# sony/NDJIR

Hardware: AMD Instinct MI355X
Metric: rays/sec (fwd+bwd) at 512 rays x 128 samples (higher is better)
Workload: dtype f32 (f16x2-split MFMA products, f32 accumulate; error vs fp64 below an fp32 FMA chain's)

## Files before the change

### include/ndjir_hip.h

```cpp
#ifndef NDJIR_HIP_H
#define NDJIR_HIP_H

#include <hip/hip_runtime_api.h>

#ifdef __cplusplus
extern "C" {
#endif

#define NDJIR_OK 0
#define NDJIR_ERR_LAUNCH 1
#define NDJIR_ERR_UNSUPPORTED 2
#define NDJIR_ERR_ARG 3

const char* ndjir_version(void);
int ndjir_zero(float* p, long long n, hipStream_t stream);

int ndjir_hash_force_align(int size, int mod);
int ndjir_hash_grid_size(int G0, float growth_factor, int level);
int ndjir_hash_table_size(int G, int T0);
long long ndjir_hash_num_params(int G0, float growth_factor, int T0, int L, int D);

#define NDJIR_DECL_VOXEL_FAMILY(P)                                                                                          \
  int ndjir_##P##_query_on_voxel(int N, float* output, const float* query, const float* feature, const int* grid_sizes,     \
                                 int D, const float* min, const float* max, int boundary_check, hipStream_t stream);       \
// ... 257 lines not shown

int ndjir_geo_encode(long long P, int M, const float* x, int nseg, const float* const* seg, const int* segC, float* e, int lde,
                     hipStream_t stream);
int ndjir_geo_normal(long long P, int M, const float* e, int lde, const float* g0, int ldg, int nseg, const float* const* gq,
                     float* n_out, float* Z, int ldz, int D, float* sdf_out, hipStream_t stream);
int ndjir_geo_backward_begin(long long P, int D, const float* g_sdf, const float* g_feat, int ldf, const float* g_n,
                             const float* gZ, int ldz, float* gy, float* nbar, hipStream_t stream);
int ndjir_geo_gbar0(long long P, int M, const float* e, int lde, const float* nbar, int nseg, const float* const* seg,
                    const int* segC, float* gb0, hipStream_t stream);
int ndjir_copy_columns(long long P, int C, const float* src, int lds, float* dst, int ldd, hipStream_t stream);
int ndjir_inverse_squared_distance(long long P, long long rows_per_batch, const float* x, int ldx, const float* camloc, float* out,
                                   int ldo, hipStream_t stream);

int ndjir_mlp_chain_group_begin(void);
int ndjir_mlp_chain_group_end(hipStream_t stream, int* launches);

#define NDJIR_MATH_FP32 0
#define NDJIR_MATH_BF16X6 1
#define NDJIR_MATH_F16X3 2
int ndjir_mlp_set_math(int math);
int ndjir_mlp_get_math(void);
int ndjir_mlp_set_tile_rows(int rows);
int ndjir_mlp_get_tile_rows(void);
int ndjir_mlp_small_affine(long long P, const float* x, int ldx, int K, const float* W, int ldw, int N, int transpose,
                           const float* bias, float* y, int ldy, hipStream_t stream);
int ndjir_mlp_set_chain_pipeline(int mask);
int ndjir_mlp_get_chain_pipeline(void);
long long ndjir_mlp_packed_size(int K, int N, int transpose);
int ndjir_mlp_pack(const float* W, float* dst, int K, int N, int transpose, hipStream_t stream);
int ndjir_mlp_pack_strided(const float* W, int ldw, float* dst, int K, int N, int transpose, hipStream_t stream);
int ndjir_mlp_pack_table(const void* table, int n, int total_blocks, hipStream_t stream);
int ndjir_mlp_pack_entry_bytes(void);
int ndjir_mlp_chain(int bwd, long long P, const float* X, int ldx, int K0, int L,
                    const float* const* Wp, const float* const* bias, const int* Ks, const int* Ns,
                    const float* const* side_in, float* const* side_out, const int* ld_side,
                    float* const* bgrad, float* Y, int ldy, int accum_y, int has_output, float beta,
                    int skip_layer, float skip_scale, int skip_split, float* Xskip, int ld_xskip,
                    float* in_bgrad, float* workspace, unsigned* const* side_amax, unsigned* x_amax, hipStream_t stream);
long long ndjir_mlp_chain_workspace(int bgrad_total);
int ndjir_mlp_chain_ex(int mode, long long P, const float* X, int ldx, int K0, int L,
                       const float* const* Wp, const float* const* bias, const int* Ks, const int* Ns,
                       const float* const* side_in, float* const* side_out, const int* ld_side,
                       float* const* bgrad, float* Y, int ldy, int accum_y, int has_output, float beta,
                       int skip_layer, float skip_scale, int skip_split, float* Xskip, int ld_xskip,
                       const float* const* side_in2, const float* const* side_add, float* const* side_out2,
                       const float* row_bias, int row_bias_div, float* in_bgrad, float* workspace,
                       unsigned* const* side_amax, unsigned* x_amax, hipStream_t stream);
int ndjir_mlp_group_colsum(const float* X, int ldx, int N, long long G, int div, float* out, int blocked, hipStream_t stream);
long long ndjir_mlp_wgrad_workspace(int K, int N, long long P);
int ndjir_mlp_wgrad(const float* A, int lda, const float* B, int ldb, int K, int N, long long P, float* out,
                    int accum, float* workspace, const unsigned* amax_a, const unsigned* amax_b, hipStream_t stream);
long long ndjir_mlp_wgrad_group_workspace(int n_src, const float* const* A, const int* lda, const long long* P, const int* out_id,
                                          int n_out, const int* K, const int* N, int target_items, const int* layout);
int ndjir_mlp_wgrad_group_launches(int n_src, const long long* P, const int* out_id, int n_out);
int ndjir_mlp_wgrad_group(int n_src, const float* const* A, const int* lda, const float* const* B, const int* ldb,
                          const long long* P, const unsigned* const* amax_a, const unsigned* const* amax_b, const int* out_id,
                          int n_out, float* const* out, const int* ldo, const int* K, const int* N, const int* accum,
                          float* workspace, int target_items, int n_extra, float* const* ex_out, const float* const* ex_partial,
                          const int* ex_n, const int* ex_S, const int* ex_stride, const int* ex_accum, const int* layout,
                          hipStream_t stream);
long long ndjir_mlp_colsum_workspace(int N, long long P);
int ndjir_mlp_colsum(const float* X, int ldx, int N, long long P, float* out, int accum, float* workspace,
                     hipStream_t stream);
int ndjir_mlp_chain_kernel(int mode, long long P, int K0, int L, const int* Ks, const int* Ns, int has_output, int skip_layer,
                           int skip_split, int with_bias_gradients, char* name, int name_bytes);
int ndjir_mlp_chain_bias_partials(int mode, long long P, int K0, int L, const int* Ks, const int* Ns, int has_output,
                                  int skip_layer, int skip_split, unsigned bgrad_mask, int in_bgrad, int* blocks, int* row_floats);
int ndjir_mlp_debug_timeline(long long* buf);


int ndjir_generate_raydir_camloc(int B, int R, const double* pose, const double* intrinsic, const int* pixel_index,
                                 const float* xy, int W, float* raydir, float* camloc, hipStream_t stream);

typedef struct ndjir_adam_state { float alpha; int t; float alpha_t; int skipped; } ndjir_adam_state;
int ndjir_solver_adam_begin(void* state, float beta1, float beta2, const int* flag_a, const int* flag_b,
                            hipStream_t stream);
int ndjir_solver_adam(long long n, float* w, float* g, float* m, float* v, float alpha_t, float beta1, float beta2,
                      float eps, float decay, int zero_grad, const void* state, hipStream_t stream);
int ndjir_solver_adam_touched(long long n, float* w, float* g, float* m, float* v, float alpha_t, float beta1, float beta2,
                              float eps, float decay, unsigned* touched, const void* state, hipStream_t stream);
int ndjir_voxel_feature_mark_touched(int N, const float* query, const int* grid_sizes, int D, const float* min,
                                     const float* max, unsigned* bitmap, hipStream_t stream);
int ndjir_solver_adam_multi(int count, float* const* w, const float* const* g, float* const* m, float* const* v,
                            const long long* numel, float alpha_t, float beta1, float beta2, float eps, float decay,
                            const void* state, hipStream_t stream);
int ndjir_solver_check_inf_or_nan(long long n, const float* g, int* flag, hipStream_t stream);
int ndjir_solver_check_inf_or_nan_multi(int count, const float* const* g, const long long* numel, int* flag,
                                        hipStream_t stream);
// ... 8 lines not shown
```

### ndjir_amd/csrc/capi_mlp.hip

```cpp
#include <hip/hip_runtime.h>
#include <stdlib.h>

#include "../../include/ndjir_hip.h"
#include "common.h"
#include "mlp.h"

using namespace ndjir;

static inline int round_up(int v, int m) { return (v + m - 1) / m * m; }

static int g_math = NDJIR_MATH_F16X3;

extern "C" int ndjir_mlp_set_math(int math) {
  if (math != NDJIR_MATH_FP32 && math != NDJIR_MATH_BF16X6 && math != NDJIR_MATH_F16X3) return NDJIR_ERR_ARG;
  g_math = math;
  return NDJIR_OK;
}

extern "C" int ndjir_mlp_get_math(void) { return g_math; }

extern "C" long long ndjir_mlp_packed_size(int K, int N, int transpose) {
  if (g_math == NDJIR_MATH_BF16X6) return packed_size6(K, N, transpose);
  if (g_math == NDJIR_MATH_F16X3) return packed_size3(K, N, transpose);
  int Kp = round_up(transpose ? N : K, 8), Np = round_up(transpose ? K : N, 32);
// ... 28 lines not shown
static thread_local GroupCall* g_group = nullptr;
static thread_local int g_group_n = 0;
static thread_local int g_group_err = NDJIR_OK;
static thread_local ChainDry* g_dry = nullptr;

static int g_tile_rows = -1;
static int tile_rows_setting() {
  if (g_tile_rows < 0) { const char* e = getenv("NDJIR_MLP_TILE"); g_tile_rows = e ? atoi(e) : 0; }
  return g_tile_rows;
}
extern "C" int ndjir_mlp_set_tile_rows(int rows) {
  if (rows != 0 && rows != 32 && rows != 64 && rows != 128) return NDJIR_ERR_ARG;
  g_tile_rows = rows;
  return NDJIR_OK;
}
extern "C" int ndjir_mlp_get_tile_rows(void) { return tile_rows_setting(); }

extern "C" int ndjir_mlp_set_chain_pipeline(int mask) {
  if (mask < 0 || mask > 7) return NDJIR_ERR_ARG;
  chain_pipeline(mask);
  return NDJIR_OK;
}
extern "C" int ndjir_mlp_get_chain_pipeline(void) { return chain_pipeline(-1); }

static int chain_impl(int bwd, long long P, const float* X, int ldx, int K0, int L,
                               const float* const* Wp, const float* const* bias, const int* Ks, const int* Ns,
                               const float* const* side_in, float* const* side_out, const int* ld_side,
                               float* const* bgrad, float* Y, int ldy, int accum_y, int has_output, float beta,
                               int skip_layer, float skip_scale, int skip_split, float* Xskip, int ld_xskip,
                               const float* const* side_in2, const float* const* side_add, float* const* side_out2,
                               const float* row_bias, int row_bias_div, float* in_bgrad, float* workspace,
                               unsigned* const* side_amax, unsigned* x_amax, hipStream_t stream) {
  if (P <= 0) {
    if (bwd != 0 && in_bgrad && K0 > 0 && hipMemsetAsync(in_bgrad, 0, (size_t)K0 * sizeof(float), stream) != hipSuccess)
      return NDJIR_ERR_LAUNCH;
    if (bwd != 0 && bgrad && Ns && L >= 1 && L <= MAX_CHAIN_LAYERS)
      for (int i = 0; i < L; ++i)
        if (bgrad[i] && hipMemsetAsync(bgrad[i], 0, (size_t)Ns[i] * sizeof(float), stream) != hipSuccess) return NDJIR_ERR_LAUNCH;
    return NDJIR_OK;
  }
  if (!X || L < 1 || L > MAX_CHAIN_LAYERS || !Wp || !Ks || !Ns) return NDJIR_ERR_ARG;
  if (has_output && !Y) return NDJIR_ERR_ARG;
  ChainArgs a{};
  const int forced = tile_rows_setting();
  a.tile_rows = forced ? forced : ((P + 63) / 64 < 256 ? 32 : 64);
  a.forced_tile = forced;
// ... 101 lines not shown
                               float* in_bgrad, float* workspace, unsigned* const* side_amax, unsigned* x_amax,
                               hipStream_t stream) {
  if (bwd != 0 && bwd != 1) return NDJIR_ERR_ARG;
  return chain_impl(bwd, P, X, ldx, K0, L, Wp, bias, Ks, Ns, side_in, side_out, ld_side, bgrad, Y, ldy, accum_y,
                    has_output, beta, skip_layer, skip_scale, skip_split, Xskip, ld_xskip, nullptr, nullptr, nullptr, nullptr, 0,
                    in_bgrad, workspace, side_amax, x_amax, stream);
}

extern "C" int ndjir_mlp_chain_ex(int mode, long long P, const float* X, int ldx, int K0, int L,
                                  const float* const* Wp, const float* const* bias, const int* Ks, const int* Ns,
                                  const float* const* side_in, float* const* side_out, const int* ld_side,
                                  float* const* bgrad, float* Y, int ldy, int accum_y, int has_output, float beta,
                                  int skip_layer, float skip_scale, int skip_split, float* Xskip, int ld_xskip,
                                  const float* const* side_in2, const float* const* side_add, float* const* side_out2,
                                  const float* row_bias, int row_bias_div, float* in_bgrad, float* workspace,
                                  unsigned* const* side_amax, unsigned* x_amax, hipStream_t stream) {
  if (mode < 0 || mode > 2) return NDJIR_ERR_ARG;
  return chain_impl(mode, P, X, ldx, K0, L, Wp, bias, Ks, Ns, side_in, side_out, ld_side, bgrad, Y, ldy, accum_y,
                    has_output, beta, skip_layer, skip_scale, skip_split, Xskip, ld_xskip, side_in2, side_add, side_out2,
                    row_bias, row_bias_div, in_bgrad, workspace, side_amax, x_amax, stream);
}

static int chain_dry(int mode, long long P, int K0, int L, const int* Ks, const int* Ns, int has_output, int skip_layer,
                     int skip_split, unsigned bgrad_mask, int in_bgrad, ChainDry* out) {
  if (mode < 0 || mode > 2 || L < 1 || L > MAX_CHAIN_LAYERS || !Ks || !Ns || P <= 0) return NDJIR_ERR_ARG;
  static float dummy[4];
  const float* wp[MAX_CHAIN_LAYERS];
  const float* side[MAX_CHAIN_LAYERS];
  float* bg[MAX_CHAIN_LAYERS];
  for (int i = 0; i < L; ++i) { wp[i] = dummy; side[i] = dummy; bg[i] = (mode != 0 && ((bgrad_mask >> i) & 1)) ? dummy : nullptr; }
  out->name[0] = 0; out->blocks = 0; out->bg_total = 0;
  g_dry = out;
  const int rc = chain_impl(mode, P, dummy, K0, K0, L, wp, nullptr, Ks, Ns, mode != 0 ? side : nullptr, nullptr, nullptr,
                            mode != 0 ? bg : nullptr, dummy, Ns[L - 1], 0, has_output, 100.f, skip_layer, 1.f,
                            skip_split, (mode == 1 && skip_layer >= 0) ? dummy : nullptr, K0, nullptr, nullptr, nullptr, nullptr, 0,
                            (mode != 0 && in_bgrad) ? dummy : nullptr, dummy, nullptr, nullptr, nullptr);
  g_dry = nullptr;
  return rc;
}

extern "C" int ndjir_mlp_chain_kernel(int mode, long long P, int K0, int L, const int* Ks, const int* Ns, int has_output,
                                      int skip_layer, int skip_split, int with_bias_gradients, char* name, int name_bytes) {
  if (!name || name_bytes < 64) return NDJIR_ERR_ARG;
  ChainDry d;
  const int rc = chain_dry(mode, P, K0, L, Ks, Ns, has_output, skip_layer, skip_split, with_bias_gradients ? ~0u : 0u, 0, &d);
  for (int i = 0; i < 64; ++i) name[i] = d.name[i];
  return rc;
}

extern "C" int ndjir_mlp_chain_bias_partials(int mode, long long P, int K0, int L, const int* Ks, const int* Ns, int has_output,
                                             int skip_layer, int skip_split, unsigned bgrad_mask, int in_bgrad, int* blocks,
                                             int* row_floats) {
  if (!blocks || !row_floats) return NDJIR_ERR_ARG;
  ChainDry d;
  const int rc = chain_dry(mode, P, K0, L, Ks, Ns, has_output, skip_layer, skip_split, bgrad_mask, in_bgrad, &d);
  if (rc != NDJIR_OK) return rc;
  if (d.bg_total < 0) return NDJIR_ERR_UNSUPPORTED;
  *blocks = d.blocks;
  *row_floats = d.bg_total;
  return NDJIR_OK;
}

extern "C" long long ndjir_mlp_chain_workspace(int bgrad_total) { return chain_workspace(bgrad_total); }

extern "C" long long ndjir_mlp_wgrad_workspace(int K, int N, long long P) { return wgrad_workspace(K, N, P); }

extern "C" int ndjir_mlp_wgrad(const float* A, int lda, const float* B, int ldb, int K, int N, long long P, float* out,
                               int accum, float* workspace, const unsigned* amax_a, const unsigned* amax_b,
// ... 63 lines not shown
```

### ndjir_amd/csrc/mlp.h

```cpp
#pragma once
#include <hip/hip_runtime.h>

namespace ndjir {

constexpr int MAX_CHAIN_LAYERS = 10;

struct ChainLayer {
  const float* Wp;
  const float* bias;
  const float* side_in;
  const float* side_in2;
  const float* side_add;
  float* side_out2;
  float* side_out;
  float* bgrad;
  unsigned* side_amax;
  int bg_off;
  int K, N;
  int Kp, Np;
  int ld_side;
};

struct ChainDry {
  char name[64];
// ... 43 lines not shown
static_assert(sizeof(ChainGroup) <= 4096, "kernel arguments are limited to 4 KB");

int launch_pack(const float* W, float* dst, int K, int N, int transpose, hipStream_t stream);
int launch_chain(const ChainArgs& a, int mode, hipStream_t stream);
int launch_bgrad_reduce(const float* partial, int S, int total, float* const* ptr, const int* off, int n, int accum, hipStream_t stream);
long long packed_size6(int K, int N, int transpose);
int launch_pack6(const float* W, float* dst, int K, int N, int transpose, hipStream_t stream);
int launch_chain6(const ChainArgs& a, int mode, hipStream_t stream);
long long packed_size3(int K, int N, int transpose);
int launch_pack3(const float* W, int ldw, float* dst, int K, int N, int transpose, hipStream_t stream);
struct PackEntry {
  const float* W;
  float* dst;
  int K, N, ldw, transpose;
  int Kp, Np;
  int first_block;
  int pad;
};
int launch_pack3_table(const PackEntry* table, int n, int total_blocks, hipStream_t stream);
int launch_chain3(const ChainArgs& a, int mode, hipStream_t stream);
int launch_chainw(const ChainArgs& a, int mode, hipStream_t stream);
int launch_chainw_group(const ChainArgs* nets, int n, int mode, hipStream_t stream);
int chain_pipeline(int set);
constexpr int CHAIN_MAX_GRID_BG = 512;
inline long long chain_workspace(int bg_total) { return (long long)CHAIN_MAX_GRID_BG * ((bg_total + 3) & ~3); }
long long wgrad_workspace(int K, int N, long long P);
int launch_wgrad(const float* A, int lda, const float* B, int ldb, int K, int N, long long P, float* out, int accum,
                 float* workspace, int math, const unsigned* amax_a, const unsigned* amax_b, hipStream_t stream);

long long wgrad_group_workspace(int n_src, const float* const* A, const int* lda, const long long* P, const int* out_id, int n_out,
                                const int* K, const int* N, int target_items, const int* layout);
int wgrad_group_launches(int n_src, const long long* P, const int* out_id, int n_out);
int launch_wgrad_group(int n_src, const float* const* A, const int* lda, const float* const* B, const int* ldb, const long long* P,
                       const unsigned* const* amax_a, const unsigned* const* amax_b, const int* out_id, int n_out,
                       float* const* out, const int* ldo, const int* K, const int* N, const int* accum, float* workspace,
                       int target_items, int n_extra, float* const* ex_out, const float* const* ex_partial, const int* ex_n,
                       const int* ex_S, const int* ex_stride, const int* ex_accum, const int* layout, hipStream_t stream);

long long colsum_workspace(int N, long long P);
int launch_group_colsum(const float* X, int ldx, int N, long long G, int div, float* out, int blocked, hipStream_t stream);
int launch_colsum(const float* X, int ldx, int N, long long P, float* out, int accum, float* workspace,
                  hipStream_t stream);

}
```

### ndjir_amd/csrc/mlp3.hip

```cpp
#include <hip/hip_runtime.h>
#include <stdio.h>
#include <stdint.h>

#include <type_traits>

#include "common.h"
#include "mlp.h"
#include "mlp3_util.h"

namespace ndjir {
namespace x3 {

using namespace x3u;

constexpr int NWAVES = 8;
constexpr int NTHREADS = NWAVES * 64;
constexpr int MAXNB = 16;
constexpr int GPS = 32 * 4 + 4;
constexpr int STG = 8 * GPS;
constexpr int IN_CACHE = 10;
#ifndef NDJIR_BWD_KLOOP_BARRIER
#define NDJIR_BWD_KLOOP_BARRIER 0
#endif
constexpr bool BWD_KLOOP_BARRIER = NDJIR_BWD_KLOOP_BARRIER;
// ... 840 lines not shown

int launch_pack3_table(const PackEntry* table, int n, int total_blocks, hipStream_t stream) {
  if (n <= 0 || total_blocks <= 0) return NDJIR_OK;
  hipLaunchKernelGGL(x3::k_pack3_table, dim3(total_blocks), dim3(x3::PACK_T), 0, stream, table, n);
  return ndjir_check_launch();
}

int launch_chain3(const ChainArgs& a, int mode, hipStream_t stream) {
  using namespace x3;
  constexpr int LDS_DYN_MAX = 160 * 1024 - 2048;
  if (a.P <= 0) return NDJIR_OK;
  if (a.tile_rows == 128 || (a.tile_rows == 64 && a.forced_tile == 0)) {
    const int rc = launch_chainw(a, mode, stream);
    if (rc != NDJIR_ERR_UNSUPPORTED) return rc;
  }
  int TM = a.tile_rows == 32 ? 32 : 64;
  int wmax = round_up(a.K0, 16);
  for (int i = 0; i < a.L; ++i) {
    const bool last = a.has_output && i == a.L - 1;
    if (a.layers[i].Np > MAXNB * 32) return NDJIR_ERR_UNSUPPORTED;
    if (!last && a.layers[i].Np > NWAVES * 32) TM = 32;
    if (!last && a.layers[i].Np > 32) { if (a.layers[i].Np > wmax) wmax = a.layers[i].Np; }
  }
  const int TMP = TM + 4;
  if (a.skip_layer >= 0 && mode != 1) { int w = round_up(a.layers[a.skip_layer].N + a.K0, 16); if (w > wmax) wmax = w; }
  ChainArgs b = a;
  b.K0p = round_up(a.K0, 16);
  b.lds_split = (wmax / 8) * TMP;
  size_t lds_bytes = (size_t)2 * b.lds_split * 16;
  size_t stage_bytes = (size_t)NWAVES * 2 * STG * 4;
  const size_t partials = (size_t)4 * TM * 32 * 4;
  if (stage_bytes < partials) stage_bytes = partials;
  lds_bytes += stage_bytes;
  b.n_tiles = (a.P + TM - 1) / TM;
  float* bg_ptr[MAX_CHAIN_LAYERS + 1];
  int bg_off[MAX_CHAIN_LAYERS + 1];
  int bg_n = 0, bg_total = 0;
  if (mode != 0) {
    for (int i = 0; i < a.L; ++i) if (a.layers[i].bgrad && !(a.has_output && i == a.L - 1)) {
      b.layers[i].bg_off = bg_total;
      bg_ptr[bg_n] = a.layers[i].bgrad;
      bg_off[bg_n] = bg_total;
      ++bg_n;
      bg_total += a.layers[i].N;
    } else b.layers[i].bgrad = nullptr;
  }
// ... 36 lines not shown
```

### ndjir_amd/lib.py

```python
import ctypes
import os

import torch

_HERE = os.path.dirname(os.path.abspath(__file__))
SO_PATH = os.environ.get("NDJIR_HIP_LIB") or os.path.join(_HERE, "_lib", "libndjir_hip.so")

_vp = ctypes.c_void_p
_CT = {"i": ctypes.c_int, "f": ctypes.c_float, "p": _vp, "q": _vp, "F": ctypes.POINTER(ctypes.c_float),
       "I": ctypes.POINTER(ctypes.c_int), "l": ctypes.c_longlong, "P": ctypes.POINTER(_vp),
       "A": ctypes.POINTER(ctypes.c_int), "L": ctypes.POINTER(ctypes.c_longlong), "x": _vp,
       "W": ctypes.POINTER(ctypes.c_float)}

_VOX_TAIL, _PLN_TAIL, _HSH_TAIL = "IiFFi", "iiFFi", "ifiiiFFi"


def _family(prefix, fwd, tail):
    return {
        f"{prefix}_{fwd}": "ippp" + tail,
        f"{prefix}_grad_query": "ipppp" + tail + "i",
        f"{prefix}_grad_feature": "ippp" + tail + "i",
        f"{prefix}_grad_query_grad_grad_output": "ipppp" + tail + "i",
        f"{prefix}_grad_query_grad_feature": "ipppp" + tail + "i",
    }
# ... 206 lines not shown
            cargs.append(v.data_ptr())
        elif c == "W":
            cargs.append((ctypes.c_float * len(v))(*[float(x) for x in v]))
        elif c == "F":
            cargs.append(_f3(v))
        elif c == "I":
            cargs.append(_i3(v))
        elif c == "f":
            cargs.append(float(v))
        else:
            cargs.append(int(v))
    stream = torch.cuda.current_stream().cuda_stream
    rc = f(*cargs, stream)
    if rc != 0:
        raise NdjirHipError(f"ndjir_{name} failed with status {rc}")


def symbols():
    return ["ndjir_" + n for n in SIGS] + ["ndjir_version", "ndjir_hash_force_align", "ndjir_hash_grid_size",
                                            "ndjir_hash_table_size", "ndjir_hash_num_params",
                                            "ndjir_mlp_packed_size", "ndjir_mlp_wgrad_workspace", "ndjir_mlp_wgrad_group_workspace", "ndjir_mlp_wgrad_group_launches", "ndjir_mlp_colsum_workspace",
                                            "ndjir_mlp_chain_workspace", "ndjir_mlp_set_math", "ndjir_mlp_get_math",
                                            "ndjir_mlp_set_tile_rows", "ndjir_mlp_get_tile_rows", "ndjir_mlp_set_chain_pipeline", "ndjir_mlp_get_chain_pipeline", "ndjir_mlp_pack_entry_bytes",
                                            "ndjir_mlp_debug_timeline", "ndjir_mlp_chain_kernel", "ndjir_mlp_chain_bias_partials", "ndjir_loss_terms_workspace",
                                            "ndjir_mlp_chain_group_begin", "ndjir_mlp_chain_group_end", "ndjir_sparse_rows_header"]


def hash_num_params(G0, growth_factor, T0, L, D):
    return int(load().ndjir_hash_num_params(int(G0), float(growth_factor), int(T0), int(L), int(D)))
```

### ndjir_amd/mlp.py

```python
import contextlib
import os
import weakref


import torch
from torch.autograd import Function
from torch.multiprocessing.reductions import StorageWeakRef as _StorageRef

from . import lib
from .registry import REG

_PACK_CACHE = REG.pack_cache

MATH_FP32, MATH_BF16X6, MATH_F16X3 = 0, 1, 2


def set_math(math):
    if lib.load().ndjir_mlp_set_math(int(math)) != 0:
        raise lib.NdjirHipError(f"unknown math mode {math}")
    _PACK_CACHE.clear()


def get_math():
    return int(lib.load().ndjir_mlp_get_math())


def set_tile_rows(rows):
    if lib.load().ndjir_mlp_set_tile_rows(int(rows)) != 0:
        raise ValueError(f"tile rows {rows}")


def get_tile_rows():
    return int(lib.load().ndjir_mlp_get_tile_rows())


def set_chain_pipeline(mask):
    if lib.load().ndjir_mlp_set_chain_pipeline(int(mask)) != 0:
        raise ValueError(f"chain pipeline mask {mask}")


def get_chain_pipeline():
    return int(lib.load().ndjir_mlp_get_chain_pipeline())


def _init_math():
    import os
    env = os.environ.get("NDJIR_MLP_MATH")
    if env:
        set_math({"fp32": MATH_FP32, "bf16x6": MATH_BF16X6, "f16x3": MATH_F16X3}[env.lower()])

PROFILE = None


def chain_kernel_symbol(mode, P, K0, Ks, Ns, has_output=True, skip_layer=-1, skip_split=0, with_bias_gradients=False):
    import ctypes
    L = len(Ks)
    buf = ctypes.create_string_buffer(64)
    f = lib.load().ndjir_mlp_chain_kernel
    f.argtypes = [ctypes.c_int, ctypes.c_longlong, ctypes.c_int, ctypes.c_int, ctypes.POINTER(ctypes.c_int), ctypes.POINTER(ctypes.c_int),
                  ctypes.c_int, ctypes.c_int, ctypes.c_int, ctypes.c_int, ctypes.c_char_p, ctypes.c_int]
    f.restype = ctypes.c_int
    rc = f(int(mode), int(P), int(K0), L, (ctypes.c_int * L)(*[int(k) for k in Ks]), (ctypes.c_int * L)(*[int(n) for n in Ns]),
           1 if has_output else 0, int(skip_layer), int(skip_split), 1 if with_bias_gradients else 0, buf, 64)
    return buf.value.decode() if rc == 0 else f"ndjir chain (status {rc})"


def _launch_symbol(name, args):
    if name in ("mlp_chain", "mlp_chain_ex"):
        return chain_kernel_symbol(args[0], args[1], args[4], args[8], args[9], bool(args[17]), args[19], args[21],
                                   any(t is not None for t in args[13]) or (args[29 if name == "mlp_chain_ex" else 24] is not None))
    if name == "mlp_wgrad_group":
        return "ndjir::k_wgrad_group_wide + k_wgrad_group (+ k_wgrad_group_reduce)"
    if name == "mlp_wgrad":
        return "ndjir::k_wgrad3 / k_wgrad_narrow (+ split reduction)"
    return "ndjir::" + name


_BIAS_ARENA = {}
_BIAS_LAYOUT = {}


def _bias_region(device, floats):
    a = _BIAS_ARENA.get(device)
    if a is None or a[1] + floats > a[0].numel():
        if torch.cuda.is_current_stream_capturing() and a is not None:
            return torch.empty(floats, device=device, dtype=torch.float32)
        t = torch.empty(max(floats, 1 << 24, a[0].numel() if a else 0), device=device, dtype=torch.float32)
        a = _BIAS_ARENA[device] = [t, 0]
    out = a[0][a[1]:a[1] + floats]
    a[1] += (floats + 3) // 4 * 4
    _held(a[0])
    return out

# ... 441 lines not shown
        return self.t.data_ptr() + 128 * self.c0

    def __getitem__(self, idx):
        rows, cols = idx
        assert rows == slice(None) and isinstance(cols, slice) and cols.step is None
        a, b, _ = cols.indices(self.c1 - self.c0)
        return PB(self.t, self.c0 + a, self.c0 + b)


def pb(t, on=True):
    return PB(t) if (on and t is not None) else t


def blocked_layout(P, hidden_widths, is_cuda=True):
    if _NO_BLOCKED or _NO_GROUP or not is_cuda or get_math() != MATH_F16X3 or P % 128 != 0:
        return False
    tile = get_tile_rows()
    if not (tile == 128 or (tile == 0 and P >= 32768)):
        return False
    return all(64 <= -(-int(w) // 32) * 32 <= 256 for w in hidden_widths)


def engine_state():
    return (get_math(), get_tile_rows(), get_chain_pipeline())


def require_engine(saved, blocked):
    if blocked and saved is not None and saved != engine_state():
        raise RuntimeError(f"ndjir_amd.mlp: the MLP engine changed between forward and backward ((math, tile_rows) {saved} -> "
                           f"{engine_state()}); set_math / set_tile_rows must not be called while a forward pass's graph "
                           f"(autograd or captured HIP graph) is alive")


def chain_workspace(device, bgrads):
    total = sum(b.numel() for b in bgrads if b is not None)
    if not total:
        return None
    need = lib.load().ndjir_mlp_chain_workspace(total)
    if _GROUP is not None:
        return torch.empty(need, device=device, dtype=torch.float32)
    return _workspace(device, need)


def chain_forward(x, weights, biases, beta=100.0, skip_layer=-1, skip_scale=1.0, keep_hidden=False, row_bias=None,
                  row_bias_div=1, K0=None, out=None, blocked=False):
    P, ldx = x.shape
    blk = 8 if (blocked and keep_hidden) else 0
# ... 412 lines not shown
                if ctx.needs_input_grad[7 + L + j]:
                    if btgt[j] is not None:
                        if j == L - 1 and gb_last is None:
                            colsum(gy2, out=btgt[j][1:] if tail else btgt[j], accum=True)
                    elif j == L - 1 and tail:
                        if gb_last is None:
                            gb_full = torch.zeros((gy2.shape[1] + 1,), device=x2.device, dtype=torch.float32)
                            colsum(gy2, out=gb_full[1:])
                        gb[j] = gb_full
                    else:
                        gb[j] = bgrads[j] if j < L - 1 else (gb_last if gb_last is not None else colsum(gy2))
        g_rb = None
        rb_shape, rb_div = ctx.rb
        if rb_shape is not None and ctx.needs_input_grad[1]:
            d0 = deltas[0]
            G = P // rb_div
            g_rb = torch.empty((G, d0.shape[1]), device=d0.device, dtype=torch.float32)
            lib.call("mlp_group_colsum", _Strided(d0), d0.stride(0), d0.shape[1], G, rb_div, g_rb, 1 if (blk and L > 1) else 0)
            g_rb = g_rb.view(rb_shape)
        return (gx.reshape(xshape) if gx is not None else None, g_rb, None, None, None, None, None, *gW, *gb)


def fused_mlp(x, weights, biases, beta=100.0, skip_layer=-1, skip_scale=1.0, row_bias=None, row_bias_div=1, pack=None):
    return FusedMLP.apply(x, row_bias, row_bias_div, beta, skip_layer, skip_scale, pack, *weights, *biases)


class MultiMLP(Function):

    @staticmethod
    def forward(ctx, x, beta, net_cfg, lazy_pad, *params):
        ld = x.shape[-1]
        x2 = x.detach().reshape(-1, ld).contiguous()
        train = any(ctx.needs_input_grad)
        per_net, off = [], 0
        for L, K0, div in net_cfg:
            rb = None
            if div > 0:
                rb = params[off].detach().reshape(-1, params[off].shape[-1])
                off += 1
            per_net.append((rb, list(params[off:off + L]), list(params[off + L:off + 2 * L])))
            off += 2 * L
        res = [None] * len(net_cfg)
        blks = [False] * len(net_cfg)
        with chain_group():
            for n in sorted(range(len(net_cfg)), key=lambda i: (_width_class(per_net[i][1]), i)):
                (L, K0, div), (rb, W, b) = net_cfg[n], per_net[n]
# ... 283 lines not shown
```

Before: 69040.

## Add persistent small-tile forward chain kernel with register weight prefetch ring

```diff
diff --git a/include/ndjir_hip.h b/include/ndjir_hip.h
--- a/include/ndjir_hip.h
+++ b/include/ndjir_hip.h
@@ -303,6 +303,8 @@
 int ndjir_mlp_get_math(void);
 int ndjir_mlp_set_tile_rows(int rows);
 int ndjir_mlp_get_tile_rows(void);
+int ndjir_mlp_set_chain_small(int mask);
+int ndjir_mlp_get_chain_small(void);
 int ndjir_mlp_small_affine(long long P, const float* x, int ldx, int K, const float* W, int ldw, int N, int transpose,
                            const float* bias, float* y, int ldy, hipStream_t stream);
 int ndjir_mlp_set_chain_pipeline(int mask);
@@ -345,6 +347,8 @@
                      hipStream_t stream);
 int ndjir_mlp_chain_kernel(int mode, long long P, int K0, int L, const int* Ks, const int* Ns, int has_output, int skip_layer,
                            int skip_split, int with_bias_gradients, char* name, int name_bytes);
+int ndjir_mlp_chain_kernel_ex(int mode, long long P, int K0, int L, const int* Ks, const int* Ns, int has_output, int skip_layer,
+                              int skip_split, int with_bias_gradients, int side_outputs, char* name, int name_bytes);
 int ndjir_mlp_chain_bias_partials(int mode, long long P, int K0, int L, const int* Ks, const int* Ns, int has_output,
                                   int skip_layer, int skip_split, unsigned bgrad_mask, int in_bgrad, int* blocks, int* row_floats);
 int ndjir_mlp_debug_timeline(long long* buf);
diff --git a/ndjir_amd/csrc/capi_mlp.hip b/ndjir_amd/csrc/capi_mlp.hip
--- a/ndjir_amd/csrc/capi_mlp.hip
+++ b/ndjir_amd/csrc/capi_mlp.hip
@@ -74,6 +74,13 @@
   return NDJIR_OK;
 }
 extern "C" int ndjir_mlp_get_chain_pipeline(void) { return chain_pipeline(-1); }
+
+extern "C" int ndjir_mlp_set_chain_small(int mask) {
+  if (mask < 0 || mask > 3) return NDJIR_ERR_ARG;
+  chain_small(mask);
+  return NDJIR_OK;
+}
+extern "C" int ndjir_mlp_get_chain_small(void) { return chain_small(-1); }
 
 static int chain_impl(int bwd, long long P, const float* X, int ldx, int K0, int L,
                                const float* const* Wp, const float* const* bias, const int* Ks, const int* Ns,
@@ -221,7 +228,7 @@
 }
 
 static int chain_dry(int mode, long long P, int K0, int L, const int* Ks, const int* Ns, int has_output, int skip_layer,
-                     int skip_split, unsigned bgrad_mask, int in_bgrad, ChainDry* out) {
+                     int skip_split, unsigned bgrad_mask, int in_bgrad, ChainDry* out, int side_outputs = 0) {
   if (mode < 0 || mode > 2 || L < 1 || L > MAX_CHAIN_LAYERS || !Ks || !Ns || P <= 0) return NDJIR_ERR_ARG;
   static float dummy[4];
   const float* wp[MAX_CHAIN_LAYERS];
@@ -230,7 +237,9 @@
   for (int i = 0; i < L; ++i) { wp[i] = dummy; side[i] = dummy; bg[i] = (mode != 0 && ((bgrad_mask >> i) & 1)) ? dummy : nullptr; }
   out->name[0] = 0; out->blocks = 0; out->bg_total = 0;
   g_dry = out;
-  const int rc = chain_impl(mode, P, dummy, K0, K0, L, wp, nullptr, Ks, Ns, mode != 0 ? side : nullptr, nullptr, nullptr,
+  float* sout[MAX_CHAIN_LAYERS];
+  for (int i = 0; i < L; ++i) sout[i] = dummy;
+  const int rc = chain_impl(mode, P, dummy, K0, K0, L, wp, nullptr, Ks, Ns, mode != 0 ? side : nullptr, side_outputs ? sout : nullptr, nullptr,
                             mode != 0 ? bg : nullptr, dummy, Ns[L - 1], 0, has_output, 100.f, skip_layer, 1.f,
                             skip_split, (mode == 1 && skip_layer >= 0) ? dummy : nullptr, K0, nullptr, nullptr, nullptr, nullptr, 0,
                             (mode != 0 && in_bgrad) ? dummy : nullptr, dummy, nullptr, nullptr, nullptr);
@@ -243,6 +252,16 @@
   if (!name || name_bytes < 64) return NDJIR_ERR_ARG;
   ChainDry d;
   const int rc = chain_dry(mode, P, K0, L, Ks, Ns, has_output, skip_layer, skip_split, with_bias_gradients ? ~0u : 0u, 0, &d);
+  for (int i = 0; i < 64; ++i) name[i] = d.name[i];
+  return rc;
+}
+
+extern "C" int ndjir_mlp_chain_kernel_ex(int mode, long long P, int K0, int L, const int* Ks, const int* Ns, int has_output,
+                                         int skip_layer, int skip_split, int with_bias_gradients, int side_outputs, char* name,
+                                         int name_bytes) {
+  if (!name || name_bytes < 64) return NDJIR_ERR_ARG;
+  ChainDry d;
+  const int rc = chain_dry(mode, P, K0, L, Ks, Ns, has_output, skip_layer, skip_split, with_bias_gradients ? ~0u : 0u, 0, &d, side_outputs);
   for (int i = 0; i < 64; ++i) name[i] = d.name[i];
   return rc;
 }
diff --git a/ndjir_amd/csrc/mlp.h b/ndjir_amd/csrc/mlp.h
--- a/ndjir_amd/csrc/mlp.h
+++ b/ndjir_amd/csrc/mlp.h
@@ -89,6 +89,8 @@
 int launch_chainw(const ChainArgs& a, int mode, hipStream_t stream);
 int launch_chainw_group(const ChainArgs* nets, int n, int mode, hipStream_t stream);
 int chain_pipeline(int set);
+int launch_chain3s(const ChainArgs& a, int mode, int TM, hipStream_t stream);
+int chain_small(int set);
 constexpr int CHAIN_MAX_GRID_BG = 512;
 inline long long chain_workspace(int bg_total) { return (long long)CHAIN_MAX_GRID_BG * ((bg_total + 3) & ~3); }
 long long wgrad_workspace(int K, int N, long long P);
diff --git a/ndjir_amd/csrc/mlp3.hip b/ndjir_amd/csrc/mlp3.hip
--- a/ndjir_amd/csrc/mlp3.hip
+++ b/ndjir_amd/csrc/mlp3.hip
@@ -886,6 +886,10 @@
     if (!last && a.layers[i].Np > NWAVES * 32) TM = 32;
     if (!last && a.layers[i].Np > 32) { if (a.layers[i].Np > wmax) wmax = a.layers[i].Np; }
   }
+  if (mode == 0) {
+    const int rc = launch_chain3s(a, mode, TM, stream);
+    if (rc != NDJIR_ERR_UNSUPPORTED) return rc;
+  }
   const int TMP = TM + 4;
   if (a.skip_layer >= 0 && mode != 1) { int w = round_up(a.layers[a.skip_layer].N + a.K0, 16); if (w > wmax) wmax = w; }
   ChainArgs b = a;
diff --git a/ndjir_amd/csrc/mlp3s.hip b/ndjir_amd/csrc/mlp3s.hip
--- /dev/null
+++ b/ndjir_amd/csrc/mlp3s.hip
@@ -0,0 +1,445 @@
+#include <hip/hip_runtime.h>
+#include <stdio.h>
+#include <stdint.h>
+#include <stdlib.h>
+
+#include <type_traits>
+#include <utility>
+
+#include "common.h"
+#include "mlp.h"
+#include "mlp3_util.h"
+
+namespace ndjir {
+namespace x3 {
+
+using namespace x3u;
+
+namespace small {
+constexpr int NWAVES = 8;
+constexpr int NTHREADS = NWAVES * 64;
+constexpr int MAXNB = 16;
+constexpr int MAXHB = 8;
+constexpr int KSPLIT = 4;
+constexpr int RING = 8;
+
+template <class F, int... J>
+__device__ __forceinline__ void for_each_slot(F&& f, std::integer_sequence<int, J...>) { (f(std::integral_constant<int, J>{}), ...); }
+
+struct Layout {
+  int xkeep;
+  int part;
+  int bias;
+  int winv;
+  int bias_stride;
+};
+}
+
+template <int TM>
+__global__ void __launch_bounds__(small::NTHREADS, 1) k_chain3s(ChainArgs a, small::Layout lo) {
+  using namespace small;
+  constexpr int RB = TM / 32;
+  constexpr int TMP = TM + 4;
+  extern __shared__ __attribute__((aligned(16))) float lds[];
+  __shared__ unsigned s_rmax[2][64];
+  __shared__ unsigned s_xmax[2][64];
+  __shared__ float s_ainv[64];
+  const int PLANE = a.lds_split;
+  f16x8* act = reinterpret_cast<f16x8*>(lds);
+  char* actb = reinterpret_cast<char*>(lds);
+  float* xkeep = lds + lo.xkeep;
+  float* part = lds + lo.part;
+  float* lbias = lds + lo.bias;
+  float* lwinv = lds + lo.winv;
+  const int tid = threadIdx.x;
+  const int lane = tid & 63;
+  const int wave = __builtin_amdgcn_readfirstlane(tid >> 6);
+  auto fresh_lane = [&]() { int l = lane; asm volatile("" : "+v"(l)); return l; };
+  const float beta = a.beta;
+  const float b2 = beta * LOG2E;
+  const int L = a.L;
+  const int K0 = a.K0, K0p = a.K0p;
+
+  auto put4 = [&](int k, int m, f32x4 v, float s) {
+    f16x4 ph, pl;
+    split4(v, s, ph, pl);
+    char* p = actb + ((size_t)((k >> 3) * TMP + m) * 16 + (k & 7) * 2);
+    *reinterpret_cast<f16x4*>(p) = ph;
+    *reinterpret_cast<f16x4*>(p + (size_t)PLANE * 16) = pl;
+  };
+  auto put1 = [&](int k, int m, float v, float s) {
+    _Float16 ph, pl;
+    split1(v, s, ph, pl);
+    char* p = actb + ((size_t)((k >> 3) * TMP + m) * 16 + (k & 7) * 2);
+    *reinterpret_cast<_Float16*>(p) = ph;
+    *reinterpret_cast<_Float16*>(p + (size_t)PLANE * 16) = pl;
+  };
+
+  struct Seg { gptr<const f16x8> base; int k0, k1; };
+  auto n_pass = [&](int li) { const int NB = a.layers[li].Np >> 5; return NB == 1 ? 1 : (NB + NWAVES - 1) / NWAVES; };
+  auto seg_of = [&](int li, int pass) {
+    const ChainLayer& ly = a.layers[li];
+    const int KS = (ly.Kp + 15) >> 4, NB = ly.Np >> 5;
+    Seg s;
+    int nb = 0;
+    if (NB == 1) {
+      const int kq = wave;
+      const bool on = kq < KSPLIT;
+      s.k0 = on ? (KS * kq) / KSPLIT : 0;
+      s.k1 = on ? (KS * (kq + 1)) / KSPLIT : 0;
+    } else {
+      nb = wave + NWAVES * pass;
+      s.k0 = 0;
+      s.k1 = nb < NB ? KS : 0;
+      if (nb >= NB) nb = 0;
+    }
+    s.base = (gptr<const f16x8>)reinterpret_cast<const f16x8*>(ly.Wp) + (long long)nb * KS * 2 * 64;
+    return s;
+  };
+
+  for (int li = wave; li < L; li += NWAVES) {
+    const ChainLayer& ly = a.layers[li];
+    const int KS = (ly.Kp + 15) >> 4, NB = ly.Np >> 5;
+    for (int i = lane; i < lo.bias_stride; i += 64) lbias[li * lo.bias_stride + i] = (ly.bias && i < ly.N) ? ly.bias[i] : 0.f;
+    if (lane < MAXNB) lwinv[li * MAXNB + lane] = lane < NB ? (ly.Wp + (long long)KS * 16 * ly.Np)[lane] : 0.f;
+  }
+  if (tid < 128) { (&s_rmax[0][0])[tid] = 0u; (&s_xmax[0][0])[tid] = 0u; }
+
+  gptr<const f16x8> pf_base = (gptr<const f16x8>)reinterpret_cast<const f16x8*>(a.layers[0].Wp);
+  int pf_k = 0, pf_k1 = 1;
+  int pf_li = 0, pf_pass = -1;
+  long long pf_tiles = (a.n_tiles - (long long)blockIdx.x + (long long)gridDim.x - 1) / (long long)gridDim.x;
+  bool pf_valid = false;
+  for (int li = 0; li < L; ++li)
+    for (int p = 0, np = n_pass(li); p < np; ++p) { const Seg s = seg_of(li, p); if (s.k0 < s.k1) pf_valid = true; }
+  if (pf_tiles <= 0) pf_valid = false;
+  auto pf_next_seg = [&]() {
+    while (pf_valid) {
+      if (++pf_pass >= n_pass(pf_li)) {
+        pf_pass = 0;
+        if (++pf_li >= L) { pf_li = 0; if (--pf_tiles <= 0) { pf_valid = false; break; } }
+      }
+      const Seg s = seg_of(pf_li, pf_pass);
+      if (s.k0 < s.k1) { pf_base = s.base; pf_k = s.k0; pf_k1 = s.k1; break; }
+    }
+  };
+  auto pf_advance = [&]() {
+    if (!pf_valid) return;
+    if (pf_k + RING < pf_k1) pf_k += RING; else pf_next_seg();
+  };
+
+  f16x8 ring[RING][2];
+  f32x16 acc0[RB], acc1[RB];
+  auto ring_fill = [&](auto jtag, const int lane_k) {
+    constexpr int J = decltype(jtag)::value;
+    const int ks = pf_k + J < pf_k1 ? pf_k + J : pf_k;
+#pragma unroll
+    for (int p = 0; p < 2; ++p) ring[J][p] = pf_base[(long long)(ks * 2 + p) * 64 + lane_k];
+  };
+  auto chunk = [&](const int k, const int nvalid) {
+    const int lane_k = fresh_lane();
+    const f16x8* A0 = act + (lane_k >> 5) * TMP + (lane_k & 31) + 2 * k * TMP;
+    f16x8 af[2][2][RB];
+#pragma unroll
+    for (int q = 0; q < RB; ++q) { af[0][0][q] = A0[q * 32]; af[0][1][q] = A0[PLANE + q * 32]; }
+    auto step = [&](auto jtag) {
+      constexpr int J = decltype(jtag)::value;
+      constexpr int C = J & 1;
+      if (J + 1 < RING && J + 1 < nvalid) {
+        const f16x8* An = A0 + 2 * (J + 1) * TMP;
+#pragma unroll
+        for (int q = 0; q < RB; ++q) { af[C ^ 1][0][q] = An[q * 32]; af[C ^ 1][1][q] = An[PLANE + q * 32]; }
+      }
+      if (J < nvalid) {
+#pragma unroll
+        for (int q = 0; q < RB; ++q) acc1[q] = __builtin_amdgcn_mfma_f32_32x32x16_f16(ring[J][0], af[C][1][q], acc1[q], 0, 0, 0);
+#pragma unroll
+        for (int q = 0; q < RB; ++q) acc0[q] = __builtin_amdgcn_mfma_f32_32x32x16_f16(ring[J][0], af[C][0][q], acc0[q], 0, 0, 0);
+#pragma unroll
+        for (int q = 0; q < RB; ++q) acc1[q] = __builtin_amdgcn_mfma_f32_32x32x16_f16(ring[J][1], af[C][0][q], acc1[q], 0, 0, 0);
+      }
+      ring_fill(jtag, lane_k);
+      __builtin_amdgcn_sched_barrier(0);
+    };
+    for_each_slot(step, std::make_integer_sequence<int, RING>{});
+    pf_advance();
+  };
+
+  pf_next_seg();
+  {
+    const int lane_k = fresh_lane();
+    for_each_slot([&](auto jtag) { ring_fill(jtag, lane_k); }, std::make_integer_sequence<int, RING>{});
+  }
+  pf_advance();
+  __syncthreads();
+  int xpar = 0;
+
+  for (long long tile = blockIdx.x; tile < a.n_tiles; tile += gridDim.x) {
+    const long long row0 = tile * TM;
+    const int rows = (int)((a.P - row0) < TM ? (a.P - row0) : TM);
+
+    {
+      const float* X = a.X + row0 * a.ldx;
+      const int groups = K0p >> 2;
+      const int total = groups * TM;
+      const bool vec = (a.ldx & 3) == 0 && ((uintptr_t)a.X & 15) == 0;
+      for (int t = tid; t < total; t += NTHREADS) {
+        const int g = t % groups, m = t / groups;
+        const int k = g * 4;
+        f32x4 v = {0.f, 0.f, 0.f, 0.f};
+        if (m < rows) {
+          if (vec && k + 3 < K0) v = *reinterpret_cast<const f32x4*>(X + (long long)m * a.ldx + k);
+          else {
+#pragma unroll
+            for (int q = 0; q < 4; ++q) if (k + q < K0) v[q] = X[(long long)m * a.ldx + k + q];
+          }
+        }
+        unsigned mb = 0;
+#pragma unroll
+        for (int q = 0; q < 4; ++q) { const unsigned b = finite_abs_bits(v[q]); mb = b > mb ? b : mb; }
+        if (mb) atomicMax(&s_xmax[xpar][m], mb);
+        *reinterpret_cast<f32x4*>(xkeep + m * K0p + k) = v;
+      }
+      __syncthreads();
+      if (tid < TM) {
+        float s_row, inv_row;
+        scale_from_max(s_xmax[xpar][tid], s_row, inv_row);
+        s_ainv[tid] = inv_row;
+        s_xmax[xpar ^ 1][tid] = 0u;
+      }
+      for (int t = tid; t < total; t += NTHREADS) {
+        const int g = t % groups, m = t / groups;
+        const int k = g * 4;
+        float s_in, inv_in;
+        scale_from_max(s_xmax[xpar][m], s_in, inv_in);
+        put4(k, m, *reinterpret_cast<const f32x4*>(xkeep + m * K0p + k), s_in);
+      }
+    }
+    __syncthreads();
+
+    int cur = 0;
+#pragma unroll 1
+    for (int li = 0; li < L; ++li) {
+      const ChainLayer& ly = a.layers[li];
+      const int NB = ly.Np >> 5;
+      const bool last = li == L - 1;
+      const int l_N = ly.N;
+      const bool has_bias = ly.bias != nullptr;
+      const bool is_skip = (li == a.skip_layer);
+      const float sc = is_skip ? a.skip_scale : 1.f;
+      const float ib2sc = LN2 / beta * sc;
+      const float* const bias_l = lbias + li * lo.bias_stride;
+      const float* const winv_l = lwinv + li * MAXNB;
+
+      const bool narrow = NB == 1;
+      const bool active = narrow ? wave < KSPLIT : wave < NB;
+
+      const int np = narrow ? 1 : (NB + NWAVES - 1) / NWAVES;
+#pragma unroll 1
+      for (int pass = 0; pass < np; ++pass) {
+        const Seg s = seg_of(li, pass);
+#pragma unroll
+        for (int q = 0; q < RB; ++q) { acc0[q] = f32x16{0}; acc1[q] = f32x16{0}; }
+#pragma unroll 1
+        for (int k = s.k0; k < s.k1; k += RING) chunk(k, s.k1 - k < RING ? s.k1 - k : RING);
+        const int nb = wave + NWAVES * pass;
+        if (!last || narrow || nb >= NB) continue;
+        const int lane_o = fresh_lane();
+        const int r_o = lane_o & 31, hh = lane_o >> 5;
+        const int fb = nb * 32 + 4 * hh;
+        const float winv = winv_l[nb];
+#pragma unroll
+        for (int J = 0; J < RB; ++J) {
+          const int R = J * 32 + r_o;
+          if (R >= rows) continue;
+          const float sa = s_ainv[R];
+          float* y = a.Y + (row0 + R) * a.ldy + fb;
+#pragma unroll
+          for (int g = 0; g < 4; ++g) {
+            const f32x4 b4 = *reinterpret_cast<const f32x4*>(bias_l + fb + 8 * g);
+#pragma unroll
+            for (int q = 0; q < 4; ++q) {
+              if (fb + 8 * g + q >= l_N) continue;
+              float t = out_add(out_z(acc_sum(acc0[J][4 * g + q], acc1[J][4 * g + q]), sa, winv), has_bias ? b4[q] : 0.f);
+              if (a.accum_y) t = out_add(t, y[8 * g + q]);
+              y[8 * g + q] = t;
+            }
+          }
+        }
+      }
+
+      if (narrow) {
+        if (active) {
+          const int lane_o = fresh_lane();
+          const int r_o = lane_o & 31, hh = lane_o >> 5;
+#pragma unroll
+          for (int J = 0; J < RB; ++J) {
+            float* dst = part + ((size_t)(wave * TM + J * 32 + r_o)) * 32 + 4 * hh;
+#pragma unroll
+            for (int g = 0; g < 4; ++g) {
+              f32x4 v;
+#pragma unroll
+              for (int q = 0; q < 4; ++q) v[q] = acc_sum(acc0[J][4 * g + q], acc1[J][4 * g + q]);
+              *reinterpret_cast<f32x4*>(dst + 8 * g) = v;
+            }
+          }
+        }
+        __syncthreads();
+        const float winv = winv_l[0];
+        for (int t = tid; t < TM * 32; t += NTHREADS) {
+          const int n = t & 31, m = t >> 5;
+          float z = 0.f;
+#pragma unroll
+          for (int q = 0; q < KSPLIT; ++q) z += part[q * TM * 32 + t];
+          z = out_z(z, s_ainv[m], winv);
+          if (n < l_N && m < rows) {
+            z = out_add(z, has_bias ? bias_l[n] : 0.f);
+            float* y = a.Y + (row0 + m) * a.ldy + n;
+            *y = a.accum_y ? out_add(z, *y) : z;
+          }
+        }
+        __syncthreads();
+        continue;
+      }
+      if (last) {
+        __syncthreads();
+        continue;
+      }
+
+      if (active) {
+        const int lane_o = fresh_lane();
+        const int r_o = lane_o & 31, hh = lane_o >> 5;
+        const int fb = wave * 32 + 4 * hh;
+        const float winv = winv_l[wave];
+        f32x4 bb[4];
+#pragma unroll
+        for (int g = 0; g < 4; ++g) {
+          const f32x4 b4 = *reinterpret_cast<const f32x4*>(bias_l + fb + 8 * g);
+#pragma unroll
+          for (int q = 0; q < 4; ++q) bb[g][q] = has_bias ? b4[q] * b2 : 0.f;
+        }
+#pragma unroll
+        for (int J = 0; J < RB; ++J) {
+          const int R = J * 32 + r_o;
+          const bool mrow = R < rows;
+          const float kk = fwd_kk(s_ainv[R], winv, b2);
+          float m = 0.f;
+#pragma unroll
+          for (int i = 0; i < 16; ++i) {
+            const int f = fb + (i & 3) + 8 * (i >> 2);
+            const float u = fwd_u(acc_sum(acc0[J][i], acc1[J][i]), kk, bb[i >> 2][i & 3]);
+            const float v = (f < l_N && mrow) ? softplus_u(u, ib2sc) : 0.f;
+            acc0[J][i] = v;
+            m = fmaxf(m, fabsf(v));
+          }
+          if (!(m < 3.0e38f)) {
+            unsigned mb = 0;
+#pragma unroll
+            for (int i = 0; i < 16; ++i) { const unsigned b = finite_abs_bits(acc0[J][i]); mb = b > mb ? b : mb; }
+            m = __uint_as_float(mb);
+          }
+          atomicMax(&s_rmax[cur][R], __float_as_uint(m));
+        }
+      }
+      if (is_skip && tid < TM) {
+        const float xm = __uint_as_float(s_xmax[xpar][tid]) * fabsf(a.skip_scale);
+        atomicMax(&s_rmax[cur][tid], __float_as_uint(xm));
+      }
+      __syncthreads();
+
+      if (active) {
+        const int lane_o = fresh_lane();
+        const int r_o = lane_o & 31, hh = lane_o >> 5;
+        const int fb = wave * 32 + 4 * hh;
+#pragma unroll
+        for (int J = 0; J < RB; ++J) {
+          const int R = J * 32 + r_o;
+          float s_row, inv_row;
+          scale_from_max(s_rmax[cur][R], s_row, inv_row);
+#pragma unroll
+          for (int g = 0; g < 4; ++g)
+            put4(fb + 8 * g, R, f32x4{acc0[J][4 * g], acc0[J][4 * g + 1], acc0[J][4 * g + 2], acc0[J][4 * g + 3]}, s_row);
+        }
+      }
+      if (tid < TM) {
+        float s_row, inv_row;
+        scale_from_max(s_rmax[cur][tid], s_row, inv_row);
+        s_ainv[tid] = inv_row;
+      }
+      if (is_skip) {
+        __syncthreads();
+        const int base = l_N;
+        for (int t = tid; t < K0 * TM; t += NTHREADS) {
+          const int k = t % K0, m = t / K0;
+          const float v = (m < rows) ? xkeep[m * K0p + k] * a.skip_scale : 0.f;
+          float s_row, inv_row;
+          scale_from_max(s_rmax[cur][m], s_row, inv_row);
+          put1(base + k, m, v, s_row);
+        }
+        const int wcat = base + K0, wpad = (wcat + 15) & ~15;
+        for (int t = tid; t < (wpad - wcat) * TM; t += NTHREADS) put1(wcat + t % (wpad - wcat), t / (wpad - wcat), 0.f, 1.f);
+      }
+      __syncthreads();
+      if (tid < TM) s_rmax[cur][tid] = 0u;
+      cur ^= 1;
+    }
+    xpar ^= 1;
+  }
+}
+
+}
+
+constexpr int CHAIN_SMALL_DEFAULT = 3;
+static int g_chain_small = -1;
+int chain_small(int set) {
+  if (set >= 0) g_chain_small = set & 3;
+  if (g_chain_small < 0) { const char* e = getenv("NDJIR_CHAIN_SMALL"); g_chain_small = e ? (atoi(e) & 3) : CHAIN_SMALL_DEFAULT; }
+  return g_chain_small;
+}
+
+int launch_chain3s(const ChainArgs& a, int mode, int TM, hipStream_t stream) {
+  using namespace x3;
+  using namespace x3::small;
+  constexpr int LDS_DYN_MAX = 160 * 1024 - 2048;
+  auto round_up = [](int v, int m) { return (v + m - 1) / m * m; };
+  if (mode != 0 || (TM != 32 && TM != 64) || !(chain_small(-1) & (TM == 32 ? 1 : 2))) return NDJIR_ERR_UNSUPPORTED;
+  if (!a.has_output || a.row_bias || a.x_amax || a.timeline || a.L < 1 || a.K0 < 1) return NDJIR_ERR_UNSUPPORTED;
+  if (a.skip_layer >= a.L - 1) return NDJIR_ERR_UNSUPPORTED;
+  int wmax = round_up(a.K0, 16), bias_stride = 32;
+  for (int i = 0; i < a.L; ++i) {
+    const ChainLayer& ly = a.layers[i];
+    const bool last = i == a.L - 1;
+    if (ly.side_out || ly.side_amax) return NDJIR_ERR_UNSUPPORTED;
+    if (ly.Np > (last ? MAXNB : MAXHB) * 32 || (!last && ly.Np <= 32)) return NDJIR_ERR_UNSUPPORTED;
+    if (!last && ly.Np > wmax) wmax = ly.Np;
+    if (ly.Np > bias_stride) bias_stride = ly.Np;
+  }
+  if (a.skip_layer >= 0) { const int w = round_up(a.layers[a.skip_layer].N + a.K0, 16); if (w > wmax) wmax = w; }
+  const int TMP = TM + 4;
+  ChainArgs b = a;
+  b.K0p = round_up(a.K0, 16);
+  b.lds_split = (wmax / 8) * TMP;
+  b.n_tiles = (a.P + TM - 1) / TM;
+  Layout lo;
+  size_t floats = (size_t)2 * b.lds_split * 4;
+  lo.xkeep = (int)floats; floats += (size_t)TM * b.K0p;
+  lo.part = (int)floats; floats += (size_t)KSPLIT * TM * 32;
+  lo.bias = (int)floats; floats += (size_t)a.L * bias_stride;
+  lo.winv = (int)floats; floats += (size_t)a.L * MAXNB;
+  lo.bias_stride = bias_stride;
+  const size_t lds_bytes = floats * 4;
+  if (lds_bytes > (size_t)LDS_DYN_MAX) return NDJIR_ERR_UNSUPPORTED;
+  long long blocks = b.n_tiles < 256 ? b.n_tiles : 256;
+  static bool attr_set = false;
+  if (!attr_set) {
+    (void)hipFuncSetAttribute(reinterpret_cast<const void*>(&k_chain3s<32>), hipFuncAttributeMaxDynamicSharedMemorySize, LDS_DYN_MAX);
+    (void)hipFuncSetAttribute(reinterpret_cast<const void*>(&k_chain3s<64>), hipFuncAttributeMaxDynamicSharedMemorySize, LDS_DYN_MAX);
+    attr_set = true;
+  }
+  if (a.dry) { snprintf(a.dry->name, 64, "ndjir::x3::k_chain3s<%d>", TM); a.dry->blocks = (int)blocks; a.dry->bg_total = 0; return NDJIR_OK; }
+  if (TM == 32) hipLaunchKernelGGL((k_chain3s<32>), dim3((unsigned)blocks), dim3(NTHREADS), lds_bytes, stream, b, lo);
+  else hipLaunchKernelGGL((k_chain3s<64>), dim3((unsigned)blocks), dim3(NTHREADS), lds_bytes, stream, b, lo);
+  return ndjir_check_launch();
+}
+
+}
diff --git a/ndjir_amd/lib.py b/ndjir_amd/lib.py
--- a/ndjir_amd/lib.py
+++ b/ndjir_amd/lib.py
@@ -252,7 +252,7 @@
                                             "ndjir_mlp_packed_size", "ndjir_mlp_wgrad_workspace", "ndjir_mlp_wgrad_group_workspace", "ndjir_mlp_wgrad_group_launches", "ndjir_mlp_colsum_workspace",
                                             "ndjir_mlp_chain_workspace", "ndjir_mlp_set_math", "ndjir_mlp_get_math",
                                             "ndjir_mlp_set_tile_rows", "ndjir_mlp_get_tile_rows", "ndjir_mlp_set_chain_pipeline", "ndjir_mlp_get_chain_pipeline", "ndjir_mlp_pack_entry_bytes",
-                                            "ndjir_mlp_debug_timeline", "ndjir_mlp_chain_kernel", "ndjir_mlp_chain_bias_partials", "ndjir_loss_terms_workspace",
+                                            "ndjir_mlp_debug_timeline", "ndjir_mlp_chain_kernel", "ndjir_mlp_chain_kernel_ex", "ndjir_mlp_set_chain_small", "ndjir_mlp_get_chain_small","ndjir_mlp_chain_bias_partials", "ndjir_loss_terms_workspace",
                                             "ndjir_mlp_chain_group_begin", "ndjir_mlp_chain_group_end", "ndjir_sparse_rows_header"]
 
 
diff --git a/ndjir_amd/mlp.py b/ndjir_amd/mlp.py
--- a/ndjir_amd/mlp.py
+++ b/ndjir_amd/mlp.py
@@ -41,6 +41,15 @@
 
 def get_chain_pipeline():
     return int(lib.load().ndjir_mlp_get_chain_pipeline())
+
+
+def set_chain_small(mask):
+    if lib.load().ndjir_mlp_set_chain_small(int(mask)) != 0:
+        raise ValueError(f"chain small mask {mask}")
+
+
+def get_chain_small():
+    return int(lib.load().ndjir_mlp_get_chain_small())
 
 
 def _init_math():
@@ -52,23 +61,25 @@
 PROFILE = None
 
 
-def chain_kernel_symbol(mode, P, K0, Ks, Ns, has_output=True, skip_layer=-1, skip_split=0, with_bias_gradients=False):
+def chain_kernel_symbol(mode, P, K0, Ks, Ns, has_output=True, skip_layer=-1, skip_split=0, with_bias_gradients=False,
+                        side_outputs=False):
     import ctypes
     L = len(Ks)
     buf = ctypes.create_string_buffer(64)
-    f = lib.load().ndjir_mlp_chain_kernel
+    f = lib.load().ndjir_mlp_chain_kernel_ex
     f.argtypes = [ctypes.c_int, ctypes.c_longlong, ctypes.c_int, ctypes.c_int, ctypes.POINTER(ctypes.c_int), ctypes.POINTER(ctypes.c_int),
-                  ctypes.c_int, ctypes.c_int, ctypes.c_int, ctypes.c_int, ctypes.c_char_p, ctypes.c_int]
+                  ctypes.c_int, ctypes.c_int, ctypes.c_int, ctypes.c_int, ctypes.c_int, ctypes.c_char_p, ctypes.c_int]
     f.restype = ctypes.c_int
     rc = f(int(mode), int(P), int(K0), L, (ctypes.c_int * L)(*[int(k) for k in Ks]), (ctypes.c_int * L)(*[int(n) for n in Ns]),
-           1 if has_output else 0, int(skip_layer), int(skip_split), 1 if with_bias_gradients else 0, buf, 64)
+           1 if has_output else 0, int(skip_layer), int(skip_split), 1 if with_bias_gradients else 0, 1 if side_outputs else 0, buf, 64)
     return buf.value.decode() if rc == 0 else f"ndjir chain (status {rc})"
 
 
 def _launch_symbol(name, args):
     if name in ("mlp_chain", "mlp_chain_ex"):
         return chain_kernel_symbol(args[0], args[1], args[4], args[8], args[9], bool(args[17]), args[19], args[21],
-                                   any(t is not None for t in args[13]) or (args[29 if name == "mlp_chain_ex" else 24] is not None))
+                                   any(t is not None for t in args[13]) or (args[29 if name == "mlp_chain_ex" else 24] is not None),
+                                   side_outputs=args[11] is not None and any(t is not None for t in args[11]))
     if name == "mlp_wgrad_group":
         return "ndjir::k_wgrad_group_wide + k_wgrad_group (+ k_wgrad_group_reduce)"
     if name == "mlp_wgrad":
@@ -556,7 +567,7 @@
 
 
 def engine_state():
-    return (get_math(), get_tile_rows(), get_chain_pipeline())
+    return (get_math(), get_tile_rows(), get_chain_pipeline(), get_chain_small())
 
 
 def require_engine(saved, blocked):
@@ -1015,6 +1026,10 @@
 
 
 def fused_mlp(x, weights, biases, beta=100.0, skip_layer=-1, skip_scale=1.0, row_bias=None, row_bias_div=1, pack=None):
+    if not torch.is_grad_enabled():
+        det = lambda t: t.detach() if torch.is_tensor(t) else t
+        x, row_bias, pack = det(x), det(row_bias), det(pack)
+        weights, biases = [det(w) for w in weights], [det(b) for b in biases]
     return FusedMLP.apply(x, row_bias, row_bias_div, beta, skip_layer, skip_scale, pack, *weights, *biases)
 
 
```

After: 69750, median of 6. 1.01x the previous value.
